# micknoise/Maximilian

Measured on AMD Instinct MI355X. Metric: Msamples/s (voice-bank render), higher is better.
Workload: dtype f64; 1 GPU; configs[1]: 65536-voice maxiOsc::sinebuf bank, block 512, out[n][v] stored, 8 rotated buffers; voices_per_gpu=65536, block=512, parallelism=units sharded x1, mixdown=off

## Files before the change

### maximilian_amd/csrc/mxg_osc.h

```cpp
#pragma once
#if defined(__HIPCC__)
#include "mxg_common.h"
#include "mxg_sincos.h"
#else
#include <math.h>
#include <stddef.h>
#include "../../include/maxigpu.h"
#include "mxg_sincos.h"
namespace mxg {
constexpr double kChandiv = 1.0;
}
#endif

namespace mxg {
namespace {

struct OscPre {
    double inc;
    double k;
    double p1;
    double p2;
    SinTabK sk;
};

template <int WF>
__device__ __forceinline__ OscPre osc_pre(double f, double sr, double p1, double p2) {
    OscPre q;
    q.k = 0.0;
    q.p1 = p1;
    q.p2 = p2;
    q.sk = {1.0 / 120, 1.0 / 24};
    if constexpr (WF == MXG_OSC_SINEBUF) {
        q.inc = 512. / (sr / (f * kChandiv));
    } else if constexpr (WF == MXG_OSC_SINEBUF4) {
        q.inc = 512. / (sr / (f));
    } else if constexpr (WF == MXG_OSC_SAW) {
        q.inc = (1. / (sr / (f))) * 2.0;
    } else if constexpr (WF == MXG_OSC_SAWN) {
        q.inc = (1. / (sr / (f)));
        q.k = (8820.22 / f);
    } else if constexpr (WF == MXG_OSC_PHASORBETWEEN) {
        q.inc = ((p2 - p1) / (sr / (f)));
    } else if constexpr (WF == MXG_OSC_PULSE) {
        double duty = p1;
        if (duty < 0.) duty = 0;
        if (duty > 1.) duty = 1;
        q.p1 = duty;
        q.inc = (1. / (sr / (f)));
    } else {
        q.inc = (1. / (sr / (f)));
    }
    return q;
}

template <bool UNIT = false>
__device__ __forceinline__ double wrap_at_one(double phase) {
#if defined(__HIP_DEVICE_COMPILE__)
    if constexpr (UNIT) return __builtin_amdgcn_fract(phase);
    return phase - __hiloint2double(phase >= 1.0 ? 0x3FF00000 : 0, 0);
#else
    return phase >= 1.0 ? phase - 1.0 : phase;
#endif
}

template <bool FAST>
__device__ __forceinline__ double wrap_at_511(double phase) {
#if defined(__HIP_DEVICE_COMPILE__)
    if constexpr (FAST) return phase - __hiloint2double(phase >= 511 ? 0x40800000 : 0, 0);
#endif
    if (phase >= 511) phase -= 512;
    return phase;
}

#ifndef MXG_SB4_PAIRS
#define MXG_SB4_PAIRS 0
#endif
constexpr int kTickLean = 3;
template <int WF, int FL>
constexpr int tab_copy() {
    return (FL & 1) ? (WF == MXG_OSC_SINEBUF ? 520 : (WF == MXG_OSC_SAWN ? 1008 : 0)) : 0;
}
constexpr int kSb4Copy = 520;
constexpr int kSineOddOff = 515;
template <int WF, bool TRUST = false, int FL = 0>
__device__ __forceinline__ double osc_tick(double &phase, double &hold, const OscPre &q,
                                           const double *s_sine, const double *s_trans) {
    if constexpr (WF == MXG_OSC_SINEWAVE) {
        double r = sin_2pi_phase<TRUST>(phase, s_sine, q.sk);
        hold = r;
        phase = wrap_at_one<TRUST>(phase);
        phase += q.inc;
        return r;
    } else if constexpr (WF == MXG_OSC_COSWAVE) {
        double r = cos_2pi_phase<TRUST>(phase, s_sine, q.sk);
        hold = r;
        phase = wrap_at_one<TRUST>(phase);
        phase += q.inc;
        return r;
    } else if constexpr (WF == MXG_OSC_PHASOR) {
        double r = phase;
        hold = r;
        if (phase >= 1.0) phase -= 1.0;
        phase += q.inc;
        return r;
    } else if constexpr (WF == MXG_OSC_SAW) {
        double r = phase;
        hold = r;
        if (phase >= 1.0) phase -= 2.0;
        phase += q.inc;
        return r;
    } else if constexpr (WF == MXG_OSC_TRIANGLE) {
        if (phase >= 1.0) phase -= 1.0;
        phase += q.inc;
        const double t = (phase <= 0.5) ? phase : (1.0 - phase);
        const double r = (t - 0.25) * 4;
        hold = r;
        return r;
    } else if constexpr (WF == MXG_OSC_SQUARE) {
        if (phase < 0.5) hold = -1;
        if (phase > 0.5) hold = 1;
        if (phase >= 1.0) phase -= 1.0;
        phase += q.inc;
        return hold;
    } else if constexpr (WF == MXG_OSC_PULSE) {
        if (phase >= 1.0) phase -= 1.0;
        phase += q.inc;
        if (phase < q.p1) hold = -1.;
        if (phase > q.p1) hold = 1.;
        return hold;
    } else if constexpr (WF == MXG_OSC_IMPULSE) {
        if (phase >= 1.0) phase -= 1.0;
        double r = phase < q.inc ? 1.0 : 0.0;
        phase += q.inc;
        return r;
    } else if constexpr (WF == MXG_OSC_PHASORBETWEEN) {
        double r = phase;
        hold = r;
        if (phase < q.p1) phase = q.p1;
        if (phase >= q.p2) phase = q.p1;
        phase += q.inc;
        return r;
    } else if constexpr (WF == MXG_OSC_SINEBUF) {
        phase += q.inc;
        phase = wrap_at_511<(FL & 2) != 0>(phase);
        double remainder = phase - floor(phase);
        int i = (int)phase;
        double r = (1 - remainder) * s_sine[1 + i + 1] + remainder * s_sine[2 + i + 1 + tab_copy<WF, FL>()];
        hold = r;
        return r;
    } else if constexpr (WF == MXG_OSC_SINEBUF4) {
        phase += q.inc;
        phase = wrap_at_511<true>(phase);
        double remainder = phase - floor(phase);
        int i = (int)phase;
#if defined(__HIP_DEVICE_COMPILE__) && MXG_SB4_PAIRS
        typedef double pair2 __attribute__((ext_vector_type(2)));
        const double *t = s_sine + i + (i & 1) * kSineOddOff;
        const pair2 ab = *reinterpret_cast<const pair2 *>(t), cd = *reinterpret_cast<const pair2 *>(t + 2);
        double a = ab.x;
        if (__builtin_expect(phase == 0, 0)) a = s_sine[513];
        const double b = ab.y, c = cd.x, d = cd.y;
#elif defined(__HIP_DEVICE_COMPILE__)
        const double *t = s_sine + i;
        double a = t[0];
        const double b = t[kSb4Copy + 1], c = t[2 * kSb4Copy + 2], d = t[3 * kSb4Copy + 3];
#ifndef MXG_SB4_BRANCH
#define MXG_SB4_BRANCH 0
#endif
#if MXG_SB4_BRANCH
        if (__builtin_expect(__any(phase == 0), 0)) {
            if (phase == 0) a = s_sine[513];
        }
#else
        a = (phase == 0) ? s_sine[513] : a;
#endif
#else
        int ia = (phase == 0) ? 512 : i - 1;
        double a = s_sine[ia + 1];
        double b = s_sine[i + 1];
        double c = s_sine[i + 1 + 1];
        double d = s_sine[i + 2 + 1];
#endif
        double a1 = 0.5 * (c - a);
        double a2 = a - 2.5 * b + 2. * c - 0.5 * d;
        double a3 = 0.5 * (d - a) + 1.5 * (b - c);
        double r = ((a3 * remainder + a2) * remainder + a1) * remainder + b;
        hold = r;
        return r;
    } else {
        if (phase >= 0.5) phase -= 1.0;
        phase += q.inc;
        double temp = q.k * phase;
        if (temp < -0.5) temp = -0.5;
        if (temp > 0.5) temp = 0.5;
        temp *= 1000.0;
        temp += 500.0;
        double remainder = temp - floor(temp);
        int i = (int)temp;
        double r = ((1.0 - remainder) * s_trans[i] + remainder * s_trans[1 + i + tab_copy<WF, FL>()]) - phase;
        hold = r;
        return r;
    }
}

template <int WF>
constexpr bool osc_has_pipe() {
    return WF == MXG_OSC_SINEBUF || WF == MXG_OSC_SAWN;
}
template <int K>
struct OscPipe {
    int idx[K];
    double rem[K], aux[K];
    double t0[K], t1[K];
};
template <int WF, int K, int HALF>
__device__ __forceinline__ void osc_pipe_phase_half(double &phase, const OscPre &q, OscPipe<K> &p) {
#pragma unroll
    for (int i = HALF * (K / 2); i < (HALF + 1) * (K / 2); i++) {
        if constexpr (WF == MXG_OSC_SINEBUF) {
            phase += q.inc;
            phase = wrap_at_511<true>(phase);
            p.rem[i] = phase - floor(phase);
            p.idx[i] = (int)phase + 2;
        } else {
            if (phase >= 0.5) phase -= 1.0;
            phase += q.inc;
            double temp = q.k * phase;
            if (temp < -0.5) temp = -0.5;
            if (temp > 0.5) temp = 0.5;
            temp *= 1000.0;
            temp += 500.0;
            p.rem[i] = temp - floor(temp);
            p.idx[i] = (int)temp;
            p.aux[i] = phase;
        }
    }
}
template <int WF, int K>
__device__ __forceinline__ void osc_pipe_phase(double &phase, const OscPre &q, OscPipe<K> &p) {
    osc_pipe_phase_half<WF, K, 0>(phase, q, p);
    osc_pipe_phase_half<WF, K, 1>(phase, q, p);
}
template <int WF, int K, int FL = kTickLean>
__device__ __forceinline__ void osc_pipe_fetch(OscPipe<K> &p, const double *s_tab) {
#if defined(__HIP_DEVICE_COMPILE__)
    if constexpr ((FL & 4) != 0) {
        typedef __attribute__((address_space(3))) const double lds_cd;
        unsigned eight = 8;
        asm volatile("" : "+v"(eight));
#pragma unroll
        for (int i = 0; i < K; i++) {
            lds_cd *a = (lds_cd *)(s_tab + p.idx[i]);
            p.t0[i] = *a;
            p.t1[i] = *(lds_cd *)(uintptr_t)((unsigned)(uintptr_t)a + eight);
        }
        return;
    }
#endif
    const double *s_next = s_tab + 1 + tab_copy<WF, FL>();
#pragma unroll
    for (int i = 0; i < K; i++) {
        p.t0[i] = s_tab[p.idx[i]];
        p.t1[i] = s_next[p.idx[i]];
    }
}
template <int WF, int K>
__device__ __forceinline__ void osc_pipe_finish(const OscPipe<K> &p, double (&r)[K], double &hold) {
#pragma unroll
    for (int i = 0; i < K; i++) {
        if constexpr (WF == MXG_OSC_SINEBUF)
            r[i] = (1 - p.rem[i]) * p.t0[i] + p.rem[i] * p.t1[i];
        else
            r[i] = ((1.0 - p.rem[i]) * p.t0[i] + p.rem[i] * p.t1[i]) - p.aux[i];
    }
    hold = r[K - 1];
}

template <int WF, int K>
__device__ __forceinline__ void osc_tick_chunk(double &phase, double &hold, const OscPre &q, const double *s_sine,
                                               const double *s_trans, double (&r)[K]) {
#if defined(__HIP_DEVICE_COMPILE__)
    if constexpr (osc_has_pipe<WF>()) {
        OscPipe<K> p;
        osc_pipe_phase<WF, K>(phase, q, p);
        __builtin_amdgcn_sched_barrier(0);
        osc_pipe_fetch<WF, K>(p, WF == MXG_OSC_SINEBUF ? s_sine : s_trans);
        __builtin_amdgcn_sched_barrier(0);
        osc_pipe_finish<WF, K>(p, r, hold);
        return;
    }
#endif
#pragma unroll
    for (int i = 0; i < K; i++) r[i] = osc_tick<WF, false, kTickLean>(phase, hold, q, s_sine, s_trans);
}

template <int WF>
__device__ __forceinline__ void osc_skip(double &phase, double &hold, const OscPre &q, const double *s_sine,
                                         const double *s_trans) {
    if constexpr (WF == MXG_OSC_SINEWAVE || WF == MXG_OSC_COSWAVE || WF == MXG_OSC_PHASOR || WF == MXG_OSC_TRIANGLE) {
        phase = wrap_at_one(phase);
        phase += q.inc;
    } else if constexpr (WF == MXG_OSC_SAW) {
        if (phase >= 1.0) phase -= 2.0;
        phase += q.inc;
    } else if constexpr (WF == MXG_OSC_PHASORBETWEEN) {
        if (phase < q.p1) phase = q.p1;
        if (phase >= q.p2) phase = q.p1;
        phase += q.inc;
    } else if constexpr (WF == MXG_OSC_SINEBUF || WF == MXG_OSC_SINEBUF4) {
        phase += q.inc;
        phase = wrap_at_511<true>(phase);
    } else if constexpr (WF == MXG_OSC_SAWN) {
        if (phase >= 0.5) phase -= 1.0;
        phase += q.inc;
    } else {
        (void)osc_tick<WF>(phase, hold, q, s_sine, s_trans);
    }
}

}
}
```

### maximilian_amd/csrc/mxg_pace.h

```cpp
#pragma once
#include "mxg_common.h"

namespace mxg {
namespace {

constexpr int kPaceWords = 8;
constexpr unsigned kPaceWindow = 32, kPaceLatesUp = 4, kPaceLatesDown = 1;
constexpr unsigned kPaceGaveUp = 0xffffffffu;

struct Pace {
    unsigned P, t0, k, late, cheap;
    __device__ __forceinline__ static unsigned now() { return (unsigned)__builtin_amdgcn_s_memrealtime(); }
    __device__ __forceinline__ void start(const unsigned *ctl, unsigned arg) {
        P = arg;
        if (ctl) {
            const unsigned p = __hip_atomic_load(ctl, __ATOMIC_RELAXED, __HIP_MEMORY_SCOPE_AGENT);
            if (p == kPaceGaveUp) P = 0;
            else if (p) P = p < 2 * arg ? p : 2 * arg;
        }
        k = late = cheap = 0;
        t0 = P ? now() : 0;
    }
    __device__ __forceinline__ void wait(bool is_cheap) {
        if (P) {
            const unsigned due = t0 + k * P;
            int d = (int)(now() - due);
            while (d < 0) {
                __builtin_amdgcn_s_sleep(1);
                d = (int)(now() - due);
            }
            late = (unsigned)d;
            k++;
            cheap += is_cheap ? 1u : 0u;
        }
    }
    __device__ __forceinline__ void finish(unsigned *ctl, unsigned arg, unsigned wg, unsigned nwg, bool tolerant = false) const {
        if (!ctl || !P || (wg & 15u)) return;
        const unsigned nrep = (nwg + 15u) / 16u;
        unsigned long long *acc = reinterpret_cast<unsigned long long *>(ctl + 4);
        const unsigned long long mine = ((unsigned long long)(late < 8 * P ? late : 8 * P) << 32) | ((unsigned long long)(k && cheap * 8 >= k * 7 ? 1u : 0u) << 16) | 1ull;
        const unsigned long long all = atomicAdd(acc, mine) + mine;
        if ((unsigned)(all & 0xffffu) != nrep) return;
        atomicExch(acc, 0ull);
        const unsigned worst = (unsigned)(all >> 32) / nrep, bound = (unsigned)((all >> 16) & 0xffffu);
        const unsigned c1 = atomicAdd(&ctl[1], 0u);
        unsigned p = P, w = c1 & 0xff, lates = (c1 >> 8) & 0xff, booted = (c1 >> 16) & 0xff, strikes = c1 >> 24;
        const unsigned up = tolerant ? 2 * kPaceLatesUp : kPaceLatesUp, down = tolerant ? 4 * kPaceLatesDown : kPaceLatesDown;
        if (bound * 8 >= nrep * 7) {
            const bool is_late = worst > p / 2;
            if (booted != 1) {
                strikes = is_late ? strikes + 1 : 0;
                if (booted == 0) {
                    if (is_late) {
                        booted = 2;
                        strikes = 0;
                    } else if (p > arg - arg / 4 + 1) {
                        p -= 2;
                    }
                } else if (strikes >= (tolerant ? 2u : 1u)) {
                    p++;
                    booted = 1;
                } else if (!is_late && p > arg - arg / 4) {
                    p--;
                }
            } else {
                lates += is_late ? 1 : 0;
                ++w;
                if (lates >= up) {
                    p++;
                    w = lates = 0;
                } else if (w >= kPaceWindow) {
                    if (lates <= down && p > arg - arg / 4) p--;
                    w = lates = 0;
                }
            }
        }
        if (p > arg + arg / 2) p = kPaceGaveUp;
        atomicExch(&ctl[0], p);
        atomicExch(&ctl[1], w | (lates << 8) | (booted << 16) | (strikes << 24));
        atomicExch(&ctl[7], worst);
    }
};

constexpr unsigned kTrialPhase = 32, kTrialCandidates = 3, kTrialAgain = 16384 + 5 * kTrialPhase;

struct PaceTrial {
    unsigned t_begin, n, period, tag;
    __device__ __forceinline__ static unsigned candidate(unsigned arg, unsigned i) { return arg * (31u - 2u * i) / 32u; }
    __device__ __forceinline__ void start(const unsigned *T, unsigned arg, unsigned block_len) {
        t_begin = Pace::now();
        n = 0;
        period = 0;
        tag = block_len & 0xffffu;
        if (T) {
            unsigned d = __hip_atomic_load(T, __ATOMIC_RELAXED, __HIP_MEMORY_SCOPE_AGENT);
            const unsigned w1 = __hip_atomic_load(T + 1, __ATOMIC_RELAXED, __HIP_MEMORY_SCOPE_AGENT);
            n = w1 & 0xffffu;
            if ((w1 >> 16) != tag) {
                n = 0;
                d = 0;
            }
            if (d) {
                period = d >= 2 ? (d < 2 * arg ? d : 2 * arg) : 0;
            } else {
                const unsigned ph = n / kTrialPhase;
                period = (ph >= 2 && ph < 2 + kTrialCandidates) ? candidate(arg, ph - 2) : 0;
            }
        }
    }
    __device__ __forceinline__ void finish(unsigned *T, unsigned arg, unsigned wg, unsigned nwg) const {
        if (!T || (wg & 15u)) return;
        const unsigned nrep = (nwg + 15u) / 16u;
        unsigned long long *acc = reinterpret_cast<unsigned long long *>(T + 2);
        const unsigned long long all = atomicAdd(acc, 1ull) + 1ull;
        if ((unsigned)(all & 0xffffu) != nrep) return;
        atomicExch(acc, 0ull);
        unsigned d = atomicAdd(&T[0], 0u), nn = n + 1;
        if ((atomicAdd(&T[1], 0u) >> 16) != tag) d = 0;
        if (!d) {
            if (nn % kTrialPhase == 0) {
                const unsigned t_now = Pace::now(), ph = n / kTrialPhase, wall = t_now - atomicAdd(&T[8], 0u);
                atomicExch(&T[8], t_now);
                if (ph == 1) {
                    atomicExch(&T[4], wall);
                    atomicExch(&T[5], 0xffffffffu);
                    atomicExch(&T[6], 0u);
                } else if (ph >= 2) {
                    unsigned best = atomicAdd(&T[5], 0u), best_p = atomicAdd(&T[6], 0u);
                    bool done = ph + 1 == 2 + kTrialCandidates;
                    if (wall < best) {
                        best = wall;
                        best_p = candidate(arg, ph - 2);
                        atomicExch(&T[5], best);
                        atomicExch(&T[6], best_p);
                    } else {
                        done = true;
                    }
                    if (done) d = ((unsigned long long)best * 100 < (unsigned long long)atomicAdd(&T[4], 0u) * 98) ? best_p : 1u;
                }
            }
        } else if (nn >= kTrialAgain) {
            d = 0;
            nn = 0;
        }
        atomicExch(&T[0], d);
        atomicExch(&T[1], nn | (tag << 16));
    }
};

}
}
```

### maximilian_amd/csrc/osc.hip

```cpp
#include <type_traits>

#include "mxg_common.h"
#include "maxi_tables.h"
#include "mxg_sincos.h"
#include "mxg_osc.h"
#include "mxg_lanefold.h"
#include "mxg_pace.h"

namespace mxg {

namespace {

__device__ const double MAXI_SINE_TAB_D[MAXI_SINE_TAB_LEN] = MAXI_SINE_TAB_INIT;
__device__ const double MAXI_TRANS_TAB_D[MAXI_TRANS_TAB_LEN] = MAXI_TRANS_TAB_INIT;

__device__ const double MXG_SINTAB_D[MXG_SINTAB_LEN] = {MXG_SINTAB_VALUES};

template <int WF>
constexpr bool uses_sine() {
    return WF == MXG_OSC_SINEBUF || WF == MXG_OSC_SINEBUF4;
}
static_assert((kSineOddOff & 1) == 1 && kSineOddOff >= MAXI_SINE_TAB_LEN, "parity copy of the sine table");
static_assert(tab_copy<MXG_OSC_SINEBUF, 1>() >= MAXI_SINE_TAB_LEN, "sinebuf's table copy");
static_assert(tab_copy<MXG_OSC_SAWN, 1>() >= MAXI_TRANS_TAB_LEN, "sawn's table copy");
static_assert(kSb4Copy >= MAXI_SINE_TAB_LEN && (kSb4Copy - 2) * 8 > 255 * 8, "sinebuf4's table copies: disjoint, and out of a ds_read2_b64's reach");
template <int WF, int FL = 0>
constexpr int tab_len() {
    return (WF == MXG_OSC_SINEBUF4 && MXG_SB4_PAIRS) ? kSineOddOff + MAXI_SINE_TAB_LEN + 1
           : WF == MXG_OSC_SINEBUF4                  ? 4 * kSb4Copy
           : uses_sine<WF>()                         ? tab_copy<WF, FL>() + MAXI_SINE_TAB_LEN
                           : (WF == MXG_OSC_SAWN ? tab_copy<WF, FL>() + MAXI_TRANS_TAB_LEN
                                                 : ((WF == MXG_OSC_SINEWAVE || WF == MXG_OSC_COSWAVE) ? MXG_SINTAB_WIDE_LEN : 1));
}
template <int WF, int FL = 0>
__device__ __forceinline__ void load_tab(double *s_tab) {
    if constexpr (uses_sine<WF>()) {
        for (int i = threadIdx.x; i < MAXI_SINE_TAB_LEN; i += blockDim.x) {
            s_tab[i] = MAXI_SINE_TAB_D[i];
            if constexpr (WF == MXG_OSC_SINEBUF4 && MXG_SB4_PAIRS) s_tab[kSineOddOff + i] = MAXI_SINE_TAB_D[i];
            if constexpr (tab_copy<WF, FL>() != 0) s_tab[tab_copy<WF, FL>() + i] = MAXI_SINE_TAB_D[i];
            if constexpr (WF == MXG_OSC_SINEBUF4 && !MXG_SB4_PAIRS) {
                s_tab[kSb4Copy + i] = MAXI_SINE_TAB_D[i];
                s_tab[2 * kSb4Copy + i] = MAXI_SINE_TAB_D[i];
                s_tab[3 * kSb4Copy + i] = MAXI_SINE_TAB_D[i];
            }
        }
    } else if constexpr (WF == MXG_OSC_SAWN) {
        for (int i = threadIdx.x; i < MAXI_TRANS_TAB_LEN; i += blockDim.x) {
            s_tab[i] = MAXI_TRANS_TAB_D[i];
            if constexpr (tab_copy<WF, FL>() != 0) s_tab[tab_copy<WF, FL>() + i] = MAXI_TRANS_TAB_D[i];
        }
    } else if constexpr (WF == MXG_OSC_SINEWAVE || WF == MXG_OSC_COSWAVE) {
        for (int i = threadIdx.x; i < MXG_SINTAB_WIDE_LEN; i += blockDim.x) s_tab[i] = MXG_SINTAB_D[i & (MXG_SINTAB_LEN - 1)];
    }
}

template <int WF, bool FPS, int VPL, int ST, bool PX>
__global__ void osc_kernel(size_t V, size_t N, const double *__restrict__ freq,
                           const double *__restrict__ p1, const double *__restrict__ p2,
                           double *__restrict__ phase_io, double *__restrict__ hold_io,
                           double *__restrict__ out, double sr, PartSync psync, int xcd, int p1ps, int passes, size_t v_begin,
                           size_t v_end, size_t P, unsigned *__restrict__ pace_ctl, unsigned pace_arg, unsigned *__restrict__ trial) {
#ifndef MXG_K1_LEAN_MASK
#define MXG_K1_LEAN_MASK ((1 << MXG_OSC_SINEWAVE) | (1 << MXG_OSC_COSWAVE) | (1 << MXG_OSC_SINEBUF4) | (1 << MXG_OSC_SAWN))
#endif
    constexpr bool kLean = ((MXG_K1_LEAN_MASK >> WF) & 1) != 0;
    constexpr int kFL = kLean ? kTickLean : 0;
    __shared__ __attribute__((aligned(16))) double s_tab[tab_len<WF, kFL>()];
    constexpr bool kPre = tab_len<WF, kFL>() > 1;
    double ph0[VPL] = {}, hd0[VPL] = {}, f0[VPL] = {};
    if constexpr (kPre) {
        const size_t w0 = v_begin + ((size_t)xcd_block(blockIdx.x, gridDim.x, xcd) * blockDim.x + threadIdx.x) * VPL;
        const size_t wc = (w0 + VPL <= v_end) ? w0 : (v_end >= v_begin + VPL ? v_end - VPL : v_begin);
#pragma unroll
        for (int j = 0; j < VPL; j++) {
            const size_t w = wc + j < v_end ? wc + j : v_end - 1;
            ph0[j] = phase_io[w];
            hd0[j] = hold_io[w];
            f0[j] = FPS ? 0.0 : freq[w];
        }
    }
    if constexpr (tab_len<WF, kFL>() > 1) {
        load_tab<WF, kFL>(s_tab);
        __syncthreads();
    }
    for (int pass = 0; pass < passes; pass++) {
    const size_t v0 = v_begin + (((size_t)pass * gridDim.x + xcd_block(blockIdx.x, gridDim.x, xcd)) * blockDim.x + threadIdx.x) * VPL;
    if (v0 >= v_end) return;

    double ph[VPL], hd[VPL];
    OscPre q[VPL];
#pragma unroll
    for (int j = 0; j < VPL; j++) {
        const bool pre = kPre && pass == 0 && v0 + VPL <= v_end;
        ph[j] = pre ? ph0[j] : phase_io[v0 + j];
        hd[j] = pre ? hd0[j] : hold_io[v0 + j];
        double a = p1 ? p1[v0 + j] : 0.0, b = p2 ? p2[v0 + j] : 0.0;
        if constexpr (!FPS) {
            q[j] = osc_pre<WF>(pre ? f0[j] : freq[v0 + j], sr, a, b);
        } else {
            q[j].p1 = a;
            q[j].p2 = b;
        }
    }
    int *const part_ctr = gridDim.y > 1 ? part_counter(psync) : nullptr;
    if (blockIdx.y + 1 != gridDim.y) part_signal(part_ctr);
    const size_t plen = (N + gridDim.y - 1) / gridDim.y;
    const size_t nA = blockIdx.y * plen < N ? blockIdx.y * plen : N;
    const size_t nB = nA + plen < N ? nA + plen : N;
    if constexpr (!FPS) {
#pragma unroll 4
        for (size_t n = 0; n < nA; n++) {
#pragma unroll
            for (int j = 0; j < VPL; j++) osc_skip<WF>(ph[j], hd[j], q[j], s_tab, s_tab);
        }
    }
    double *o = out + nA * P + v0;
    const double *fp = freq + v0;
    const double *pp = (FPS && p1ps) ? p1 + v0 : nullptr;
#ifndef MXG_OSC_UNROLL
#define MXG_OSC_UNROLL 4
#endif

    bool trust = false;
    if constexpr ((WF == MXG_OSC_SINEWAVE || WF == MXG_OSC_COSWAVE) && !FPS) {
        bool ok = true;
#pragma unroll
        for (int j = 0; j < VPL; j++)
            ok = ok && q[j].inc >= 0.0 && q[j].inc < 1.0 && ph[j] >= 0.0 && ph[j] < 2.0 && (__double2hiint(ph[j]) | __double2hiint(q[j].inc)) >= 0;
        trust = __all(ok);
        if (trust) {
#pragma unroll
            for (int j = 0; j < VPL; j++) q[j].sk = sintab_k();
        }
    }
    PaceTrial tr;
    tr.start(trial, pace_arg, (unsigned)N);
    Pace pc;
    pc.start(trial ? nullptr : pace_ctl, trial ? tr.period : pace_arg);
    auto run = [&](auto trust_tag) {
        constexpr bool kTrust = decltype(trust_tag)::value;
        size_t n = nA;
        if constexpr (PX && VPL == 1 && !FPS) {
            double *op = out + (nA + (threadIdx.x & 1)) * P + (v0 & ~(size_t)1);
            if constexpr (!kLean) {
                if (pc.P) {
                    double *o8 = out + nA * P + v0;
                    for (; n + 8 <= nB; n += 8) {
                        pc.wait(true);
#pragma unroll
                        for (int u = 0; u < 8; u++) {
                            store1<1>(o8, osc_tick<WF, kTrust, kFL>(ph[0], hd[0], q[0], s_tab, s_tab));
                            o8 += P;
                        }
                    }
                    op += (n - nA) * P;
                }
#pragma unroll 2
                for (; n + 2 <= nB; n += 2) {
                    const double r0 = osc_tick<WF, kTrust, kFL>(ph[0], hd[0], q[0], s_tab, s_tab);
                    const double r1 = osc_tick<WF, kTrust, kFL>(ph[0], hd[0], q[0], s_tab, s_tab);
                    store_pair_rows<ST, false>(op, r0, r1);
                    op += 2 * P;
                }
            } else {
                const unsigned pairs = (unsigned)((nB - nA) >> 1);
                for (unsigned k = 0; k < pairs; k++) {
                    const double r0 = osc_tick<WF, kTrust, kFL>(ph[0], hd[0], q[0], s_tab, s_tab);
                    const double r1 = osc_tick<WF, kTrust, kFL>(ph[0], hd[0], q[0], s_tab, s_tab);
                    store_pair_rows<ST>(op, r0, r1);
                    op += 2 * P;
                }
                n = nA + 2 * (size_t)pairs;
            }
            o = out + n * P + v0;
        }
        if constexpr (VPL == 1 && !FPS && !PX && !kLean) {
            if (pc.P) {
                for (; n + 8 <= nB; n += 8) {
                    pc.wait(true);
#pragma unroll
                    for (int u = 0; u < 8; u++) {
                        store1<ST>(o, osc_tick<WF, kTrust, kFL>(ph[0], hd[0], q[0], s_tab, s_tab));
                        o += P;
                    }
                }
            }
        }
#pragma unroll MXG_OSC_UNROLL
        for (; n < nB; n++) {
            double r[VPL];
#pragma unroll
            for (int j = 0; j < VPL; j++) {
                if constexpr (FPS) q[j] = osc_pre<WF>(fp[j], sr, pp ? pp[j] : q[j].p1, q[j].p2);
                r[j] = osc_tick<WF, kTrust, kFL>(ph[j], hd[j], q[j], s_tab, s_tab);
            }
            if constexpr (VPL == 2)
                store2<ST>(o, r[0], r[1]);
            else
                store1<ST>(o, r[0]);
            o += P;
            if constexpr (FPS) {
                fp += V;
                if (pp) pp += V;
            }
        }
    };
    if constexpr ((WF == MXG_OSC_SINEWAVE || WF == MXG_OSC_COSWAVE) && !FPS) {
        if (trust) run(std::true_type{}); else run(std::false_type{});
    } else {
        run(std::false_type{});
    }
    if (blockIdx.y + 1 == gridDim.y && part_wait(part_ctr, psync)) {
#pragma unroll
        for (int j = 0; j < VPL; j++) {
            phase_io[v0 + j] = ph[j];
            hold_io[v0 + j] = hd[j];
        }
    }
    if (threadIdx.x == 0) {
        pc.finish(trial ? nullptr : pace_ctl, pace_arg, blockIdx.x, gridDim.x, WF == MXG_OSC_SINEBUF);
        tr.finish(trial, pace_arg, blockIdx.x, gridDim.x);
    }
    }
}


template <int WF, int STORE, int WIN>
__global__ __launch_bounds__(256) void osc_mix_kernel(size_t V, size_t N, const double *__restrict__ freq,
                                                      const double *__restrict__ p1, const double *__restrict__ p2,
                                                      double *__restrict__ phase_io, double *__restrict__ hold_io,
                                                      double *__restrict__ out, const double *__restrict__ pan,
                                                      double *__restrict__ partial, double sr, PartSync psync, int passes) {
    constexpr int kTab = tab_len<WF, kTickLean>();
    constexpr int kTabPad = (kTab + 1) & ~1;
    __shared__ __attribute__((aligned(16))) double s_all[kTabPad + 4 * kTileWave + 4 * WIN * 2 + 256];
    double *s_tab = s_all;
    load_tab<WF, kTickLean>(s_tab);
    const int lane = threadIdx.x & 63, wave = threadIdx.x >> 6;
    double *tile = s_all + kTabPad + wave * kTileWave;
    double *s_part = s_all + kTabPad + 4 * kTileWave;
    double *my_part = s_part + wave * (WIN * 2);
    double *s_dump = s_part + 4 * WIN * 2;
    for (int pass = 0; pass < passes; pass++) {
    const size_t wg = (size_t)pass * gridDim.x + blockIdx.x;
    if (wg * blockDim.x >= V) break;
    if (pass) __syncthreads();
    const size_t vraw = wg * blockDim.x + threadIdx.x;
    const bool live = vraw < V;
    const size_t v = live ? vraw : (STORE == 2 ? V - 2 + (vraw & 1) : V - 1);
    double ph = phase_io[v], hd = hold_io[v];
    double x = pan[v];
    if (x > 1) x = 1;
    if (x < 0) x = 0;
    const int ts = lane & 15, tq = lane >> 4;
    double gl[16], gr[16];
    tile[lane] = live ? sqrt(1.0 - x) : 0.0;
    tile[64 + lane] = live ? sqrt(x) : 0.0;
    __syncthreads();
#pragma unroll
    for (int j = 0; j < 16; j++) {
        gl[j] = tile[16 * tq + j];
        gr[j] = tile[64 + 16 * tq + j];
    }
    OscPre q = osc_pre<WF>(freq[v], sr, p1 ? p1[v] : 0.0, p2 ? p2[v] : 0.0);
    asm volatile("" : "+v"(ph), "+v"(hd));
    asm volatile("" : "+v"(q.inc), "+v"(q.k), "+v"(q.p1), "+v"(q.p2));
#pragma unroll
    for (int j = 0; j < 16; j++) asm volatile("" : "+v"(gl[j]), "+v"(gr[j]));
    __syncthreads();
    int *const part_ctr = gridDim.y > 1 ? part_counter(psync) : nullptr;
    if (blockIdx.y + 1 != gridDim.y) part_signal(part_ctr);
    const size_t plen = ((N + gridDim.y - 1) / gridDim.y + kMixChunk - 1) / kMixChunk * kMixChunk;
    const size_t nA = blockIdx.y * plen < N ? blockIdx.y * plen : N;
    const size_t nB = nA + plen < N ? nA + plen : N;
#pragma unroll 4
    for (size_t n = 0; n < nA; n++) osc_skip<WF>(ph, hd, q, s_tab, s_tab);
    double *tw = tile + tq * kTileQuarter + ts;
    const double2v *tr = reinterpret_cast<const double2v *>(tile + tq * kTileQuarter + ts * kTileRow);
    double *o = out + nA * V + v;
    double *op = out + (nA + (threadIdx.x & 1)) * V + (v & ~(size_t)1);
    for (size_t n0 = nA; n0 < nB; n0 += WIN) {
        const int span = (int)((nB - n0) < (size_t)WIN ? (nB - n0) : (size_t)WIN);
        auto tile_load = [&](double2v (&xv)[8]) {
#pragma unroll
            for (int k = 0; k < 8; k++) xv[k] = tr[k];
        };
        auto tile_products = [&](const double2v (&xv)[8], double &sl, double &sr2) {
            double pl[8], pr[8];
#pragma unroll
            for (int k = 0; k < 8; k++) {
                pl[k] = xv[k].x * gl[2 * k] + xv[k].y * gl[2 * k + 1];
                pr[k] = xv[k].x * gr[2 * k] + xv[k].y * gr[2 * k + 1];
            }
            sl = ((pl[0] + pl[1]) + (pl[2] + pl[3])) + ((pl[4] + pl[5]) + (pl[6] + pl[7]));
            sr2 = ((pr[0] + pr[1]) + (pr[2] + pr[3])) + ((pr[4] + pr[5]) + (pr[6] + pr[7]));
        };
        auto tile_fold = [&](double sl, double sr2) {
            const double t = fold32(sl, sr2);
            return fold16(t, t);
        };
        auto tile_value = [&](const double2v (&xv)[8]) {
            double sl, sr2;
            tile_products(xv, sl, sr2);
            return tile_fold(sl, sr2);
        };
        auto tile_put = [&](double t, int c0, int cnt) {
            double *dst = ((lane & 16) == 0 && ts < cnt) ? my_part + (c0 + ts) * 2 + (lane >> 5) : s_dump + threadIdx.x;
            *dst = t;
        };
        auto tile_sum = [&](const double2v (&xv)[8], int c0, int cnt) { tile_put(tile_value(xv), c0, cnt); };
        int c_first = 0;
        if constexpr (osc_has_pipe<WF>() && STORE != 1) {
            const int full = span / kMixChunk;
            if (full > 0) {
                OscPipe<kMixChunk> P;
                osc_pipe_phase<WF, kMixChunk>(ph, q, P);
                __builtin_amdgcn_sched_barrier(0);
                osc_pipe_fetch<WF, kMixChunk>(P, s_tab);
                double t_prev = 0.0;
                auto body = [&](int c, auto last_tag) {
                    constexpr bool kLast = decltype(last_tag)::value;
                    double r[kMixChunk];
                    auto S = [&](int j) {
                        if constexpr (STORE == 2) {
                            store_pair_rows<2>(op, r[2 * j], r[2 * j + 1]);
                            op += 2 * V;
                        }
                    };
                    __builtin_amdgcn_sched_barrier(0);
                    osc_pipe_finish<WF, kMixChunk>(P, r, hd);
                    __builtin_amdgcn_sched_barrier(0);
                    S(0);
#pragma unroll
                    for (int i = 0; i < kMixChunk; i++) tw[i * kTileRow] = r[i];
                    tile_put(t_prev, (c - 1) * kMixChunk, c > 0 ? kMixChunk : 0);
                    __builtin_amdgcn_fence(__ATOMIC_RELEASE, "wavefront");
                    __builtin_amdgcn_wave_barrier();
                    __builtin_amdgcn_fence(__ATOMIC_ACQUIRE, "wavefront");
                    double2v xv[8];
                    tile_load(xv);
                    __builtin_amdgcn_fence(__ATOMIC_RELEASE, "wavefront");
                    __builtin_amdgcn_wave_barrier();
                    __builtin_amdgcn_sched_barrier(0);
                    S(1);
                    __builtin_amdgcn_sched_barrier(0);
                    if constexpr (!kLast) {
                        osc_pipe_phase_half<WF, kMixChunk, 0>(ph, q, P);
                        __builtin_amdgcn_sched_barrier(0);
                        S(2);
                        __builtin_amdgcn_sched_barrier(0);
                        osc_pipe_phase_half<WF, kMixChunk, 1>(ph, q, P);
                        __builtin_amdgcn_sched_barrier(0);
                        S(3);
                        __builtin_amdgcn_sched_barrier(0);
                        osc_pipe_fetch<WF, kMixChunk>(P, s_tab);
                        __builtin_amdgcn_sched_barrier(0);
                    } else {
                        S(2);
                        S(3);
                    }
                    S(4);
                    __builtin_amdgcn_sched_barrier(0);
                    double vl, vr;
                    tile_products(xv, vl, vr);
                    __builtin_amdgcn_sched_barrier(0);
                    S(5);
                    __builtin_amdgcn_sched_barrier(0);
                    t_prev = tile_fold(vl, vr);
                    __builtin_amdgcn_sched_barrier(0);
                    S(6);
                    S(7);
                };
                for (int c = 0; c + 1 < full; c++) body(c, std::false_type{});
                body(full - 1, std::true_type{});
                tile_put(t_prev, (full - 1) * kMixChunk, kMixChunk);
                if constexpr (STORE == 2) o += (size_t)full * kMixChunk * V;
                c_first = full * kMixChunk;
            }
        }
        for (int c0 = c_first; c0 < span; c0 += kMixChunk) {
            const int cnt = (span - c0) < kMixChunk ? (span - c0) : kMixChunk;
            auto chunk = [&](auto full_tag) {
                constexpr bool kFull = decltype(full_tag)::value;
                if constexpr (kFull && STORE == 2) {
                    double r[kMixChunk];
#ifndef MXG_K1M_CHUNK
#define MXG_K1M_CHUNK 1
#endif
#if MXG_K1M_CHUNK
                    osc_tick_chunk<WF, kMixChunk>(ph, hd, q, s_tab, s_tab, r);
                    __builtin_amdgcn_sched_barrier(0);
#else
#pragma unroll
                    for (int i = 0; i < kMixChunk; i++) r[i] = osc_tick<WF, false, kTickLean>(ph, hd, q, s_tab, s_tab);
#endif
#pragma unroll
                    for (int i = 0; i < kMixChunk; i += 2) {
                        store_pair_rows<2>(op, r[i], r[i + 1]);
                        op += 2 * V;
                        tw[i * kTileRow] = r[i];
                        tw[(i + 1) * kTileRow] = r[i + 1];
                    }
                    o += (size_t)kMixChunk * V;
                } else if constexpr (kFull) {
                    double r[kMixChunk];
                    osc_tick_chunk<WF, kMixChunk>(ph, hd, q, s_tab, s_tab, r);
                    __builtin_amdgcn_sched_barrier(0);
#pragma unroll
                    for (int i = 0; i < kMixChunk; i++) {
                        if constexpr (STORE != 0) {
                            *o = r[i];
                            o += V;
                        }
                        tw[i * kTileRow] = r[i];
                    }
                } else {
#pragma unroll
                    for (int i = 0; i < kMixChunk; i++) {
                        double r = 0.0;
                        if (kFull || i < cnt) {
                            r = osc_tick<WF, false, kTickLean>(ph, hd, q, s_tab, s_tab);
                            if constexpr (STORE != 0) {
                                *o = r;
                                o += V;
                            }
                        }
                        tw[i * kTileRow] = r;
                    }
                    if constexpr (STORE == 2) op += (size_t)kMixChunk * V;
                }
                __builtin_amdgcn_fence(__ATOMIC_RELEASE, "wavefront");
                __builtin_amdgcn_wave_barrier();
                __builtin_amdgcn_fence(__ATOMIC_ACQUIRE, "wavefront");
                double2v xv[8];
                tile_load(xv);
                __builtin_amdgcn_fence(__ATOMIC_RELEASE, "wavefront");
                __builtin_amdgcn_wave_barrier();
                tile_sum(xv, c0, cnt);
            };
            if (cnt == kMixChunk) chunk(std::true_type{}); else chunk(std::false_type{});
        }
        __syncthreads();
        double *prow = partial + wg * N * 2 + n0 * 2;
        for (int i = threadIdx.x; i < span * 2; i += blockDim.x)
            prow[i] = ((s_part[i] + s_part[WIN * 2 + i]) + s_part[2 * WIN * 2 + i]) + s_part[3 * WIN * 2 + i];
        __syncthreads();
    }
    if (blockIdx.y + 1 == gridDim.y && part_wait(part_ctr, psync)) {
        phase_io[v] = ph;
        hold_io[v] = hd;
    }
    }
}

#ifndef MXG_PC_FL
#define MXG_PC_FL kTickLean
#endif
#ifndef MXG_PC_ASMX
#define MXG_PC_ASMX 1
#endif
#ifndef MXG_PC_CSLEEP
#define MXG_PC_CSLEEP 4
#endif
#ifndef MXG_PC_PRIO
#define MXG_PC_PRIO 2
#endif
constexpr int kPcFL = MXG_PC_FL;

template <int WF, int STORE, int WIN>
__global__ __launch_bounds__(512) void osc_mixpc_kernel(size_t V, size_t N, const double *__restrict__ freq,
                                                        const double *__restrict__ p1, const double *__restrict__ p2,
                                                        double *__restrict__ phase_io, double *__restrict__ hold_io,
                                                        double *__restrict__ out, const double *__restrict__ pan,
                                                        double *__restrict__ partial, double sr, int passes) {
    constexpr int kTab = tab_len<WF, kPcFL>();
    constexpr int kTabPad = (kTab + 1) & ~1;
    __shared__ __attribute__((aligned(16))) double s_all[kTabPad + 4 * kPcRing * kTileWave + 4 * WIN * 2 + 256 + 8];
    double *s_tab = s_all;
    const int lane = threadIdx.x & 63, wave = threadIdx.x >> 6;
    const bool producer = wave < 4;
    const int pw = wave & 3;
    double ph_pre = 0, hd_pre = 0, f_pre = 0, a_pre = 0, b_pre = 0;
    if (producer && (size_t)blockIdx.x * 256 < V) {
        const size_t vr = (size_t)blockIdx.x * 256 + (size_t)pw * 64 + lane;
        const size_t vv = vr < V ? vr : (STORE == 2 ? V - 2 + (vr & 1) : V - 1);
        ph_pre = phase_io[vv];
        hd_pre = hold_io[vv];
        f_pre = freq[vv];
// ... 623 lines not shown
```

Baseline: 805,100 Msamples/s.

## Compute paced 8-sample chunk before pacing wait and freeze trial verdicts

The paced store loop now computes each 8-sample chunk with the pipelined phase/fetch/finish path before the pace wait, then stores the results afterwards, so the wait overlaps with finished arithmetic instead of sitting in front of it. The chunk helper is parameterised on the lean-table flag. The pacing trial also skips its reduction once a verdict exists, only bumping a counter until it is time to re-trial. It also stops ending the candidate search at the first non-improving period, so every candidate is tried. The extra pipelined registers may raise register pressure, and the trial changes alter how the pacing period is picked.

```diff
diff --git a/maximilian_amd/csrc/mxg_osc.h b/maximilian_amd/csrc/mxg_osc.h
--- a/maximilian_amd/csrc/mxg_osc.h
+++ b/maximilian_amd/csrc/mxg_osc.h
@@ -276,7 +276,7 @@
     hold = r[K - 1];
 }
 
-template <int WF, int K>
+template <int WF, int K, int FL = kTickLean>
 __device__ __forceinline__ void osc_tick_chunk(double &phase, double &hold, const OscPre &q, const double *s_sine,
                                                const double *s_trans, double (&r)[K]) {
 #if defined(__HIP_DEVICE_COMPILE__)
@@ -284,14 +284,14 @@
         OscPipe<K> p;
         osc_pipe_phase<WF, K>(phase, q, p);
         __builtin_amdgcn_sched_barrier(0);
-        osc_pipe_fetch<WF, K>(p, WF == MXG_OSC_SINEBUF ? s_sine : s_trans);
+        osc_pipe_fetch<WF, K, FL>(p, WF == MXG_OSC_SINEBUF ? s_sine : s_trans);
         __builtin_amdgcn_sched_barrier(0);
         osc_pipe_finish<WF, K>(p, r, hold);
         return;
     }
 #endif
 #pragma unroll
-    for (int i = 0; i < K; i++) r[i] = osc_tick<WF, false, kTickLean>(phase, hold, q, s_sine, s_trans);
+    for (int i = 0; i < K; i++) r[i] = osc_tick<WF, false, FL>(phase, hold, q, s_sine, s_trans);
 }
 
 template <int WF>
diff --git a/maximilian_amd/csrc/mxg_pace.h b/maximilian_amd/csrc/mxg_pace.h
--- a/maximilian_amd/csrc/mxg_pace.h
+++ b/maximilian_amd/csrc/mxg_pace.h
@@ -86,11 +86,13 @@
 
 struct PaceTrial {
     unsigned t_begin, n, period, tag;
+    unsigned verdict;
     __device__ __forceinline__ static unsigned candidate(unsigned arg, unsigned i) { return arg * (31u - 2u * i) / 32u; }
     __device__ __forceinline__ void start(const unsigned *T, unsigned arg, unsigned block_len) {
         t_begin = Pace::now();
         n = 0;
         period = 0;
+        verdict = 0;
         tag = block_len & 0xffffu;
         if (T) {
             unsigned d = __hip_atomic_load(T, __ATOMIC_RELAXED, __HIP_MEMORY_SCOPE_AGENT);
@@ -100,6 +102,7 @@
                 n = 0;
                 d = 0;
             }
+            verdict = d;
             if (d) {
                 period = d >= 2 ? (d < 2 * arg ? d : 2 * arg) : 0;
             } else {
@@ -110,6 +113,10 @@
     }
     __device__ __forceinline__ void finish(unsigned *T, unsigned arg, unsigned wg, unsigned nwg) const {
         if (!T || (wg & 15u)) return;
+        if (verdict && n + 1 < kTrialAgain) {
+            if (wg == 0) __hip_atomic_fetch_add(&T[1], 1u, __ATOMIC_RELAXED, __HIP_MEMORY_SCOPE_AGENT);
+            return;
+        }
         const unsigned nrep = (nwg + 15u) / 16u;
         unsigned long long *acc = reinterpret_cast<unsigned long long *>(T + 2);
         const unsigned long long all = atomicAdd(acc, 1ull) + 1ull;
@@ -127,14 +134,12 @@
                     atomicExch(&T[6], 0u);
                 } else if (ph >= 2) {
                     unsigned best = atomicAdd(&T[5], 0u), best_p = atomicAdd(&T[6], 0u);
-                    bool done = ph + 1 == 2 + kTrialCandidates;
+                    const bool done = ph + 1 == 2 + kTrialCandidates;
                     if (wall < best) {
                         best = wall;
                         best_p = candidate(arg, ph - 2);
                         atomicExch(&T[5], best);
                         atomicExch(&T[6], best_p);
-                    } else {
-                        done = true;
                     }
                     if (done) d = ((unsigned long long)best * 100 < (unsigned long long)atomicAdd(&T[4], 0u) * 98) ? best_p : 1u;
                 }
diff --git a/maximilian_amd/csrc/osc.hip b/maximilian_amd/csrc/osc.hip
--- a/maximilian_amd/csrc/osc.hip
+++ b/maximilian_amd/csrc/osc.hip
@@ -53,6 +53,21 @@
     } else if constexpr (WF == MXG_OSC_SINEWAVE || WF == MXG_OSC_COSWAVE) {
         for (int i = threadIdx.x; i < MXG_SINTAB_WIDE_LEN; i += blockDim.x) s_tab[i] = MXG_SINTAB_D[i & (MXG_SINTAB_LEN - 1)];
     }
+}
+
+template <int WF, int FL, int ST>
+__device__ __forceinline__ void paced_chunk(Pace &pc, double &ph, double &hd, const OscPre &q, const double *s_tab, double *&o, size_t P) {
+    double r[8];
+    osc_tick_chunk<WF, 8, FL>(ph, hd, q, s_tab, s_tab, r);
+#pragma unroll
+    for (int u = 0; u < 8; u++) asm volatile("" : "+v"(r[u]));
+    pc.wait(true);
+#pragma unroll
+    for (int u = 0; u < 8; u++) {
+        store1<ST>(o, r[u]);
+        o += P;
+    }
+    __builtin_amdgcn_sched_barrier(0);
 }
 
 template <int WF, bool FPS, int VPL, int ST, bool PX>
@@ -146,14 +161,7 @@
             if constexpr (!kLean) {
                 if (pc.P) {
                     double *o8 = out + nA * P + v0;
-                    for (; n + 8 <= nB; n += 8) {
-                        pc.wait(true);
-#pragma unroll
-                        for (int u = 0; u < 8; u++) {
-                            store1<1>(o8, osc_tick<WF, kTrust, kFL>(ph[0], hd[0], q[0], s_tab, s_tab));
-                            o8 += P;
-                        }
-                    }
+                    for (; n + 8 <= nB; n += 8) paced_chunk<WF, kFL, 1>(pc, ph[0], hd[0], q[0], s_tab, o8, P);
                     op += (n - nA) * P;
                 }
 #pragma unroll 2
@@ -177,14 +185,7 @@
         }
         if constexpr (VPL == 1 && !FPS && !PX && !kLean) {
             if (pc.P) {
-                for (; n + 8 <= nB; n += 8) {
-                    pc.wait(true);
-#pragma unroll
-                    for (int u = 0; u < 8; u++) {
-                        store1<ST>(o, osc_tick<WF, kTrust, kFL>(ph[0], hd[0], q[0], s_tab, s_tab));
-                        o += P;
-                    }
-                }
+                for (; n + 8 <= nB; n += 8) paced_chunk<WF, kFL, ST>(pc, ph[0], hd[0], q[0], s_tab, o, P);
             }
         }
 #pragma unroll MXG_OSC_UNROLL
```

Result: faster. 827,600 Msamples/s (median of 6 runs) (+2.8%).
